# Nicholaswogan/clima

Hardware: AMD Instinct MI355X
Metric: radiate() calls/sec (higher is better)
Workload: dtype f64; 1 GPU; ModernEarth column, one Radtran%radiate call: nz=200, nw=1000 (600 IR + 600 solar bins), 8 g-points, 8 zenith angles, nk=5; config 2 of BASELINE.json; parallelism=1 GPU

## Files before the change

### clima_amd/csrc/radtran_api.hip

```cpp
#include "../../include/clima_radtran_hip.h"
#include "radtran_dev.h"

#include <rccl/rccl.h>
#include <sys/stat.h>
#include <unistd.h>
#include <ctime>

#include <algorithm>
#include <cmath>
#include <cstdio>
#include <cstdlib>
#include <chrono>
#include <cstring>
#include <functional>
#include <set>
#include <string>
#include <utility>
#include <limits>
#include <vector>

using namespace clima;

namespace {

// ... 36 lines not shown
  void alloc(size_t count) {
    release();
    n = count;
    if (count) HIPCHK(hipMalloc((void **)&p, count * sizeof(T)));
  }
  bool reserve(size_t count) {
    const bool grow = n < count;
    if (grow) alloc(count);
    return grow;
  }
  void upload(const std::vector<T> &v) {
    if (!(p && owned && n == v.size())) alloc(v.size());
    if (!v.empty()) HIPCHK(hipMemcpy(p, v.data(), v.size() * sizeof(T), hipMemcpyHostToDevice));
  }
  void zero(hipStream_t s = nullptr) {
    if (n) HIPCHK(hipMemsetAsync(p, 0, n * sizeof(T), s));
  }
  void release() {
    if (p && owned) (void)hipFree(p);
    p = nullptr;
    n = 0;
    owned = true;
  }
  ~DevBuf() { release(); }
};

template <class T>
struct PinnedBuf {
  T *p = nullptr;
  size_t n = 0;
  T *reserve(size_t count, size_t spare = 0) {
    if (n < count) {
      if (p) (void)hipHostFree(p);
      p = nullptr; n = 0;
      HIPCHK(hipHostMalloc((void **)&p, sizeof(T) * (count + spare), hipHostMallocDefault));
      n = count + spare;
    }
    return p;
  }
  ~PinnedBuf() { if (p) (void)hipHostFree(p); }
};

struct KTabHost {
  int sp, ng, nP, nT;
  std::vector<double> weights, log10P, temp, log10k;
  DevBuf<double> d_log10k, d_log10P, d_temp;
// ... 15 lines not shown
  int which = 0;
  int ind_start = 0, ind_end = -1, nw = 0;
  std::vector<double> wavl, freq;
  DevBuf<double> d_freq;
};
struct WrkObj {
  Radtran *parent = nullptr;
  int which = 0;
  DevBuf<double> fup_a, fdn_a, amean, tau_band;
};

struct BatchRun {
  int n = 0, first_call = 0, CH = 0;
  bool one_launch = false, pending = false;
  double *ISR = nullptr, *OLR = nullptr, *fluxes = nullptr;
  double *rows = nullptr;
  const double *bounds = nullptr;
  size_t bounds_count = 0;
  int nsel = 0;
  const int *spec_level = nullptr;
  double *spec[4] = {nullptr, nullptr, nullptr, nullptr};
  double *spec_host = nullptr;
  size_t spec_count = 0;
};

struct Radtran {
  unsigned magic = MAGIC;
  int state = 0;
  int nz = 0, nsp = 0, np = 0, nw = 0, ng = 0;
  std::vector<double> wavl, freq;
  std::vector<KTabHost *> k;
  std::vector<XsHost *> cia, ray, pxs;
  std::vector<PartHost *> part;
  std::vector<int> part_slot;
  bool has_cont = false;
  int LH2O = -1, cont_nT = 0;
  std::vector<double> cont_temp, cont_H2O, cont_foreign;
  DevBuf<double> d_cont_temp, d_cont_H2O, d_cont_foreign;
  std::vector<double> wbin, wbin_e, wxy;
  DevBuf<double> d_wbin, d_wbin_e, d_wbin_e_pad, d_wxy, d_freq, d_rorr_tab;
  ChannelObj ir, sol;
  WrkObj wrk_ir, wrk_sol;
  double diurnal_fac = 0.5;
  std::vector<double> zenith_u, zenith_w, surface_albedo, surface_emissivity, photons_sol;
  bool has_hard_surface = true;
  double ir_tau_min = 1.0e-6;
// ... 70 lines not shown
  DevBuf<double> d_cols_arena, d_flux_arena;
  DevBuf<double> d_prep_arena, d_opr_arena, d_res_arena;
  int batch_cols_in_flight = 64;
  BatchRun dev_batch;
  std::vector<int> spec_level;
  DevBuf<int> d_spec_level;
  DevBuf<double> d_spec_stage;
  PinnedBuf<double> h_spec;
  DevBuf<int> d_batch_nsrc;
  std::vector<int> batch_nsrc;
  hipEvent_t ev_producer = nullptr;
  bool batch_shared = true;
  int rebin_mode = 1;
  bool rebin_stream = false;
  long coop_items = 34816;
  bool fused = true;
  bool ts_block_mode = false;
  DevBuf<int> d_done;
  bool defer_integration = true;
  bool flux_ptr_taken = false;
  bool int_pending = false;
  IntegrateParams pending_ip;
  long merged_integrations = 0, standalone_integrations = 0;
  int profile = 0;
  long timer_calls = 0;
  int profile_stride = 1;
  struct Ev { hipEvent_t a, b; int id; };
  std::vector<Ev> pending;
  std::vector<hipEvent_t> pool;
  double k_ms[7] = {0, 0, 0, 0, 0, 0, 0};
  int k_n[7] = {0, 0, 0, 0, 0, 0, 0};

  ~Radtran() {
    for (auto *x : k) delete x;
    for (auto *x : cia) delete x;
    for (auto *x : ray) delete x;
    for (auto *x : pxs) delete x;
    for (auto *x : part) delete x;
    for (auto &e : pending) { (void)hipEventDestroy(e.a); (void)hipEventDestroy(e.b); }
    for (auto &e : pool) (void)hipEventDestroy(e);
    if (h_col) (void)hipHostFree(h_col);
    for (auto &e : host_registered) (void)hipHostUnregister(e.first);
    for (auto &cs : copy_streams) if (cs) (void)hipStreamDestroy(cs);
    for (auto &e : bout_ev) if (e) (void)hipEventDestroy(e);
    if (h_small) (void)hipHostFree(h_small);
    if (ev_upload) (void)hipEventDestroy(ev_upload);
    if (ev_producer) (void)hipEventDestroy(ev_producer);
    if (comm) (void)ncclCommDestroy(comm);
    if (stream) (void)hipStreamDestroy(stream);
    magic = 0;
  }
};

Radtran *as_rad(void *ptr) {
  Radtran *r = reinterpret_cast<Radtran *>(ptr);
  if (!r || r->magic != MAGIC) return nullptr;
  return r;
}

void gauss_legendre(int n, std::vector<double> &x, std::vector<double> &w) {
  x.assign(n, 0.0);
  w.assign(n, 0.0);
  for (int i = 0; i < n; i++) {
    double z = std::cos(PI * (i + 0.75) / (n + 0.5)), pp = 0.0;
    for (int it = 0; it < 100; it++) {
      double p1 = 1.0, p2 = 0.0;
      for (int j = 0; j < n; j++) {
        double p3 = p2;
        p2 = p1;
        p1 = ((2.0 * j + 1.0) * z * p2 - j * p3) / (j + 1.0);
      }
      pp = n * (z * p1 - p2) / (z * z - 1.0);
      double z1 = z;
      z = z1 - p1 / pp;
      if (std::fabs(z - z1) < 1e-16) break;
    }
    x[n - 1 - i] = z;
    w[n - 1 - i] = 2.0 / ((1.0 - z * z) * pp * pp);
  }
}
// ... 15 lines not shown
  double best1 = INFINITY, best2 = INFINITY;
  for (int i = 0; i < r->nw + 1; i++) {
    double d1 = std::fabs(wavl[0] - r->wavl[i]), d2 = std::fabs(wavl[n - 1] - r->wavl[i]);
    if (d1 < best1) { best1 = d1; ind1 = i; }
    if (d2 < best2) { best2 = d2; ind2 = i; }
  }
  const char *msg = "The wavelength bins are not compatible with the k-distribution wavelength bins.";
  if (n != ind2 - ind1 + 1) { set_err(err, msg); return false; }
  for (int i = 0; i < n; i++)
    if (!is_close(wavl[i], r->wavl[ind1 + i], 1.0e-7)) { set_err(err, msg); return false; }
  c.parent = r;
  c.which = which;
  c.nw = n - 1;
  c.wavl.assign(wavl, wavl + n);
  c.freq.resize(n);
  for (int i = 0; i < n; i++) c.freq[i] = C_LIGHT / (wavl[i] * 1.0e-9);
  c.ind_start = ind1;
  c.ind_end = ind2 - 1;
  return true;
}

void upload_fields(Radtran *r) {
  if (!r->fields_dirty) return;
  if (r->stream) HIPCHK(hipStreamSynchronize(r->stream));
  r->d_zen_u.upload(r->zenith_u);
  r->d_zen_w.upload(r->zenith_w);
  {
    std::vector<double> iu(r->zenith_u.size());
    for (size_t i = 0; i < iu.size(); i++) iu[i] = 1.0 / r->zenith_u[i];
    r->d_zen_iu.upload(iu);
  }
  r->d_albedo.upload(r->surface_albedo);
  r->d_emis.upload(r->surface_emissivity);
  r->d_photons.upload(r->photons_sol);
  r->fields_dirty = false;
}

void weight_edges_and_products(const std::vector<double> &wbin, std::vector<double> &wbin_e, std::vector<double> &wxy) {
  const int ng = (int)wbin.size();
  wbin_e.assign(ng + 1, 0.0);
  for (int i = 1; i < ng + 1; i++) wbin_e[i] = wbin[i - 1] + wbin_e[i - 1];
  wxy.assign((size_t)ng * ng, 0.0);
  for (int i = 0; i < ng; i++)
    for (int j = 0; j < ng; j++) wxy[j + (size_t)i * ng] = wbin[i] * wbin[j];
}

int rebin_mode_for(const std::vector<double> &wbin, const std::vector<double> &wbin_e, const std::vector<double> &wxy, bool stream) {
// ... 372 lines not shown
  if (r->holds.w0_stored) return;
  launch_w0_from_scat(r->d_tau.p, r->d_scat.p, r->d_w0.p, r->nw, r->ng, r->nz, r->stream);
  HIPCHK(hipGetLastError());
  r->holds.w0_formed();
}

bool refuse(const Radtran *r, const char *who, int needs, char *err, bool comm_counts = true) {
  const char *t = refused(r->holds, needs, r->shard_world, comm_counts && r->comm, r->op_lo, r->op_n);
  if (t) set_err(err, t[0] == ' ' ? std::string(who) + t : std::string(t));
  return t != nullptr;
}

bool defer_allowed(bool switch_on, int shard_world, bool has_comm, int profile, bool capturing, bool flux_ptr_taken) {
  return switch_on && shard_world == 1 && !has_comm && profile != 1 && !capturing && !flux_ptr_taken;
}
bool stream_capturing(Radtran *r) {
  hipStreamCaptureStatus st = hipStreamCaptureStatusNone;
  HIPCHK(hipStreamIsCapturing(r->stream, &st));
  return st != hipStreamCaptureStatusNone;
}
bool defer_eligible(Radtran *r) {
  return defer_allowed(r->defer_integration, r->shard_world, r->comm != nullptr, r->profile, false, r->flux_ptr_taken) && !stream_capturing(r);
}
bool resolve_pending_integration(Radtran *r, const PrepParams *prep = nullptr) {
  if (!r->int_pending) return false;
  r->int_pending = false;
  if (prep && r->profile != 1 && prep_integrate_merges(*prep, r->pending_ip) && !stream_capturing(r)) {
    launch_prep_integrate(*prep, r->pending_ip, r->stream);
    HIPCHK(hipGetLastError());
    r->merged_integrations++;
    return true;
  }
  { KernelTimer t(r, 3); launch_integrate(r->pending_ip, r->stream); HIPCHK(hipGetLastError()); t.stop(); }
  r->standalone_integrations++;
  return false;
}

void enqueue_radiate(Radtran *r, const CallBufs &b, bool compute_solar, bool compute_opacity, bool allow_fused = true, bool defer = false) {
  char why[CLIMA_ERR_LEN + 1];
  if (!compute_opacity && refuse(r, "radiate", NEED_OPACITIES, why)) throw HipFail{why};
  r->timer_calls++;
  upload_fields(r);
  const bool resident = b.kind == CALL_RESIDENT, chunk = b.kind == CALL_ARENA_CHUNK;
  const ColumnDev col = column_dev(r, b);
  TwoStreamParams ts = make_twostream_params(r, b, col, compute_solar);
  const LaunchPlan plan = plan_radiate(plan_input(r, b, compute_solar, compute_opacity, allow_fused));
  bool fused_done = false;
  if (compute_opacity) {
    const int call_id = ++r->call_id;
    const PrepParams pp = make_prep_params(r, b, col, call_id, plan.prep_clears ? &ts : nullptr);
    if (!resolve_pending_integration(r, resident && !plan.prep_clears ? &pp : nullptr)) {
      KernelTimer t(r, 0); launch_prep(pp, r->stream); HIPCHK(hipGetLastError()); t.stop();
    }

    OpacityParams op = make_opacity_params(r, b, col, plan.write_w0);
    if (plan.fused.form != TS_NONE) {
      FusedParams fp;
      std::memset(&fp, 0, sizeof(fp));
      fp.ncol = b.ncol; fp.bs = b.bs;
      fp.call_id = call_id; fp.max_spins = r->fused_max_spins;
      fp.done = b.done; fp.timeout_flag = r->d_err.p + 1;
      KernelTimer t(r, 1);
      fused_done = launch_fused(op, ts, fp, plan.fused, r->stream);
      HIPCHK(hipGetLastError());
      t.stop();
      if (!fused_done) op = make_opacity_params(r, b, col, true);
// ... 29 lines not shown
  const IntegrateParams ip = make_integrate_params(r, b, compute_solar, reduce);
  r->holds.rows_enqueued(ip.host_out != nullptr);
  if (defer && resident && !reduce && !ip.host_out && integrate_fits_one_launch(ip.nchunk) && defer_eligible(r)) {
    r->pending_ip = ip;
    r->int_pending = true;
  } else {
    KernelTimer t(r, 3); launch_integrate(ip, r->stream); HIPCHK(hipGetLastError()); t.stop();
  }
  if (reduce) {
    NCCLCHK(ncclAllReduce(r->d_small.p, r->d_small.p, r->rows.reduce_count, ncclDouble, ncclSum, r->comm, r->stream));
    r->comm_reduces++;
  }
}

bool recover_fused_timeout(Radtran *r);
void settle_device_batch(Radtran *r);
void settle_pending_batch(Radtran *r);

void fetch_small(Radtran *r) {
  settle_device_batch(r);
  if (r->holds.rows_on_host) return;
  const LevelRows &l = r->rows;
  for (int pass = 0; pass < 2; pass++) {
    if (!r->holds.rows_in_pinned)
      HIPCHK(hipMemcpyAsync(r->h_small, r->d_small.p, sizeof(double) * l.count, hipMemcpyDeviceToHost, r->stream));
    HIPCHK(hipStreamSynchronize(r->stream));
    resolve_events(r);
    if (r->comm) r->comm_status = r->h_small[l.status];
    if (!r->holds.column || !recover_fused_timeout(r)) break;
  }
  f_total_row(r->h_small, l);
  r->holds.rows_fetched();
}

bool check_dims(Radtran *r, int dim_T, int dim_P, int d1, int d2, int dim_dz, int has_p, int p1, int p2,
                int r1, int r2, const double *pdens, const double *radii, char *err) {
  if (has_p && ((pdens && !radii) || (radii && !pdens))) { set_err(err, "Both pdensities and radii must be arguments."); return false; }
  if (r->np > 0 && (!has_p || !radii)) { set_err(err, "The model contains particles but \"pdensities\" and \"radii\" are not arguments."); return false; }
  if (dim_T != r->nz) { set_err(err, "\"T\" has the wrong input dimension."); return false; }
  if (dim_P != r->nz) { set_err(err, "\"P\" has the wrong input dimension."); return false; }
  if (d1 != r->nz || d2 != r->nsp) { set_err(err, "\"densities\" has the wrong input dimension."); return false; }
  if (dim_dz != r->nz) { set_err(err, "\"dz\" has the wrong input dimension."); return false; }
  if (has_p && radii) {
    if (p1 != r->nz || p2 != r->np) { set_err(err, "\"pdensities\" has the wrong input dimension."); return false; }
    if (r1 != r->nz || r2 != r->np) { set_err(err, "\"radii\" has the wrong input dimension."); return false; }
  }
  return true;
}

void do_upload(Radtran *r, const ColumnArrays &a) {
  const int nz = r->nz;
  double *h = r->h_col;
  settle_pending_batch(r);
  if (r->upload_pending) { HIPCHK(hipEventSynchronize(r->ev_upload)); r->upload_pending = false; }
  r->nsrc = pack_column(r, h, a);
  const int *meta = reinterpret_cast<const int *>(h + r->col_layout.meta);
  bool all = (nz % 2 == 0) && r->nsrc * 2 == nz;
  for (int m = 0; m < r->nsrc && all; m++) all = (meta[1 + m] & SRC_EXACT) != 0;
  r->all_pairs_exact = all;
  if (r->h_col_dev) launch_copy(r->d_col.p, r->h_col_dev, r->col_layout.count, r->stream);
  else HIPCHK(hipMemcpyAsync(r->d_col.p, h, sizeof(double) * r->col_layout.count, hipMemcpyHostToDevice, r->stream));
  HIPCHK(hipEventRecord(r->ev_upload, r->stream));
  r->upload_pending = true;
  r->last_T.assign(a.T, a.T + nz);
  r->last_P.assign(a.P, a.P + nz);
  if (r->np > 0 && a.radii) r->last_radii.assign(a.radii, a.radii + (size_t)nz * r->np); else r->last_radii.clear();
  r->holds.uploaded(a.has_particles());
}

const char *const REPLACED_MSG = "The fused opacity/two-stream hand-off of an earlier opacity pass timed out and the column has "
                                 "been replaced since: repeat the steps from that opacity pass on.";
bool recover_fused_timeout(Radtran *r) {
  if (r->comm) {
    const double st = r->comm_status;
    if (!(st > 0.0)) return false;
    r->comm_status = 0.0;
    r->checked_timeout = r->call_id;
    if (std::fmod(st, 1024.0) > 0.0 && !r->holds.opr_from_resident_column()) throw HipFail{REPLACED_MSG};
    r->fused_fallbacks++;
    enqueue_radiate(r, resident_bufs(r), st >= 1024.0 || r->last_cs, true, false);
    return true;
  }
  const int t = r->h_errflag[1];
  if (t <= r->checked_timeout) return false;
  r->checked_timeout = r->call_id;
  const bool stale_opr = t == r->call_id, stale_sol = t == r->solar_id;
  if (!stale_opr && !stale_sol) return false;
  if (r->shard_world > 1)
    throw HipFail{"The fused opacity/two-stream hand-off timed out on a bin-sharded handle whose all-reduce is the caller's; "
                  "repeat the step (radtran_fused_set(0) selects the separate launches; with radtran_comm_init_rank the "
                  "library repeats it itself)."};
  if (stale_opr && !r->holds.opr_from_resident_column()) throw HipFail{REPLACED_MSG};
  r->fused_fallbacks++;
  enqueue_radiate(r, resident_bufs(r), stale_sol || r->last_cs, true, false);
  return true;
}

constexpr const char *OPACITY_FAILED_MSG = "Opacity computation failed in one or more wavelength bins.";
bool surface_device_error(Radtran *r, char *err) {
  const bool failed = *r->h_errflag > r->checked_id;
  r->checked_id = r->call_id;
  if (failed) set_err(err, OPACITY_FAILED_MSG);
  return failed;
}

void wait_error_words(Radtran *r) {
  HIPCHK(hipMemcpyAsync(r->h_errflag, r->d_err.p, 2 * sizeof(int), hipMemcpyDeviceToHost, r->stream));
  HIPCHK(hipStreamSynchronize(r->stream));
  resolve_events(r);
}

void settle(Radtran *r) {
  settle_device_batch(r);
  for (int pass = 0; pass < 2; pass++) {
    if (r->comm && !r->holds.rows_on_host)
      HIPCHK(hipMemcpyAsync(&r->comm_status, r->d_small.p + r->rows.status, sizeof(double), hipMemcpyDeviceToHost, r->stream));
    wait_error_words(r);
    if (!r->holds.column || !recover_fused_timeout(r)) break;
  }
}

void ready_stored_opacities(Radtran *r) {
  settle(r);
  upload_fields(r);
  ensure_w0(r);
}

void defer_err(Radtran *r, const std::string &msg) {
  if (r && r->deferred_err.empty()) r->deferred_err = msg;
// ... 321 lines not shown
  TRY
  const int nw = r->nw;
  std::vector<double> wv1(nw), row(nwv), tmp(nw);
  for (int i = 0; i < nw; i++) wv1[i] = 0.5 * (r->wavl[i + 1] + r->wavl[i]);
  std::vector<double> tab[3];
  const double *src[3] = {dtau_dz, w0, g0};
  for (auto &t : tab) t.assign((size_t)nw * nP, 0.0);
  for (int i = 0; i < nP; i++) {
    const int j = nP - 1 - i;
    for (int a = 0; a < 3; a++) {
      for (int k = 0; k < nwv; k++) row[k] = src[a][i + (size_t)k * nP];
      if (futils_interp(wv1, nwv, wv, row.data(), tmp.data()) != 0) {
        set_err(err, "Interpolation error in `set_custom_optical_properties`");
        return;
      }
      for (int l = 0; l < nw; l++) tab[a][(size_t)l * nP + j] = tmp[l];
    }
  }
  std::vector<double> lp(nP);
  for (int i = 0; i < nP; i++) lp[nP - 1 - i] = std::log10(P[i]);
  bool ok = nP >= 2;
  for (int i = 1; i < nP && ok; i++) ok = lp[i] > lp[i - 1];
  if (!ok) { set_err(err, "Interpolation initialization error in `set_custom_optical_properties`"); return; }
  HIPCHK(hipStreamSynchronize(r->stream));
  r->cust_axis = lp; r->cust_nP = nP;
  r->d_cust_axis.upload(lp); r->d_cust_dtau.upload(tab[0]); r->d_cust_w0.upload(tab[1]); r->d_cust_g0.upload(tab[2]);
  r->cust_on = true;
  CATCH(err)
}

static std::vector<std::string> split_lines(const char *s) {
  std::vector<std::string> out;
  if (!s) return out;
  std::string cur;
  for (const char *c = s; *c; c++) {
    if (*c == '\n') { out.push_back(cur); cur.clear(); } else cur.push_back(*c);
  }
  if (!cur.empty()) out.push_back(cur);
  return out;
}

void radtran_set_names(void *ptr, const char *species_names, const char *particle_names, char *err) {
  clear_err(err);
  GUARD(r, ptr, err);
  auto sp = split_lines(species_names), pa = split_lines(particle_names);
  if (r->state >= 1 && ((int)sp.size() != r->nsp || (int)pa.size() != r->np)) {
    set_err(err, "radtran_set_names: the number of names does not match the number of species / particles");
// ... 161 lines not shown
      case 8: h.results_dropped(); break;
      default: out[0] = -1; return;
    }
  }
  int k = 0;
  out[k++] = h.column; out[k++] = h.column_particles; out[k++] = (int)h.uploads;
  out[k++] = h.opr; out[k++] = h.w0_stored; out[k++] = (int)h.opr_upload; out[k++] = h.opr_lo; out[k++] = h.opr_n;
  out[k++] = h.rows_on_host; out[k++] = h.rows_in_pinned;
  for (int need : {NEED_COLUMN, NEED_OPACITIES, NEED_SPECTRUM}) out[k++] = refused(h, need, shard_world, has_comm != 0, op_lo, op_n) ? 1 : 0;
  out[k++] = h.opr_from_resident_column();
  static_assert(CLIMA_HOLDS_EVENT_N == 6 && CLIMA_HOLDS_OUT_N == 14, "the orders documented in clima_radtran_hip.h");
}
void clima_test_rebin_mode_for(const int *ng, const double *weights, const int *stream, int *mode) {
  std::vector<double> wbin(weights, weights + std::max(*ng, 0)), wbin_e, wxy;
  if (wbin.empty()) { *mode = -1; return; }
  weight_edges_and_products(wbin, wbin_e, wxy);
  *mode = rebin_mode_for(wbin, wbin_e, wxy, *stream != 0);
}
void radtran_merged_integrations_get(void *ptr, int *merged, int *standalone) {
  Radtran *r = as_rad(ptr);
  *merged = r ? (int)std::min<long>(r->merged_integrations, 2147483647L) : 0;
  *standalone = r ? (int)std::min<long>(r->standalone_integrations, 2147483647L) : 0;
}

void radtran_unset_custom_optical_properties(void *ptr) {
  Radtran *r = as_rad(ptr);
  if (r) r->cust_on = false;
}

void radtran_create_end(void *ptr, const int *num_zenith_angles, const double *surface_albedo, char *err) {
  clear_err(err);
  GUARD(r, ptr, err);
  if (r->state != 1) { set_err(err, "radtran_create_end: create_begin has not been called"); return; }
  if (r->k.empty()) { set_err(err, "There are no k-distributions, yet there must be some to compute total opacity."); return; }
  if (r->ir.nw == 0 || r->sol.nw == 0) { set_err(err, "wavelength channels are not set"); return; }
  if (*num_zenith_angles < 1) { set_err(err, "number of zenith angles must be >= 1"); return; }
  TRY
  const int nz = r->nz, nw = r->nw;
  std::vector<double> x, w;
  gauss_legendre(*num_zenith_angles, x, w);
  r->zenith_u.resize(*num_zenith_angles);
  r->zenith_w.resize(*num_zenith_angles);
  for (int i = 0; i < *num_zenith_angles; i++) {
    double mu = x[i] / 2.0 + 1.0 / 2.0;
    double ang = std::acos(mu) * 180.0 / PI;
    r->zenith_w[i] = w[i] / 2.0;
    r->zenith_u[i] = std::cos(ang * PI / 180.0);
  }
  r->surface_albedo.assign(r->sol.nw, *surface_albedo);
  r->surface_emissivity.assign(r->ir.nw, 1.0);
  if (r->photons_sol.empty()) r->photons_sol.assign(r->sol.nw, 0.0);

  int dev_count = 0;
  HIPCHK(hipGetDeviceCount(&dev_count));
  if (dev_count < 1) throw HipFail{"no HIP device available: the Radtran hot path has no CPU fallback"};
  HIPCHK(hipGetDevice(&r->device));
  HIPCHK(hipStreamCreateWithFlags(&r->stream, hipStreamNonBlocking));
  HIPCHK(hipEventCreateWithFlags(&r->ev_upload, hipEventDisableTiming));

  r->slots.clear();
  auto add_slot = [&](const double *axis_dev, const std::vector<double> &axis, int source, bool flag) {
    SlotDev s;
    s.axis = axis_dev; s.n = (int)axis.size(); s.source = source;
    s.lo = *std::min_element(axis.begin(), axis.end());
    s.hi = *std::max_element(axis.begin(), axis.end());
    s.flag_clamp = flag ? 1 : 0;
    r->slots.push_back(s);
  };
  for (auto *k : r->k) {
    k->d_log10k.upload(k->log10k); k->d_log10P.upload(k->log10P); k->d_temp.upload(k->temp);
    add_slot(k->d_log10P.p, k->log10P, 0, false);
    add_slot(k->d_temp.p, k->temp, 1, false);
  }
  r->abs_entries.clear();
  for (auto *v : {&r->cia, &r->pxs})
    for (auto *xs : *v) {
      xs->d_data.upload(xs->data);
      AbsEntry e;
      e.data = xs->d_data.p; e.nT = xs->dim ? xs->nT : 0; e.slot = 0;
      e.kind = (v == &r->cia) ? ABS_CIA : ABS_COLUMN; e.a = xs->sp1; e.b = xs->sp2 < 0 ? 0 : xs->sp2;
// ... 85 lines not shown
  r->fields_dirty = true;
  compute_shard(r);
  r->holds.rows_fetched();
  r->state = 2;
  CATCH(err)
}

void radtran_upload_column(void *ptr, const double *T_surface, const double *T, const double *P,
                           const double *densities, const double *dz, const double *pdensities,
                           const double *radii, char *err) {
  clear_err(err);
  GUARD_BUILT(r, ptr, err);
  if (r->np > 0 && (!pdensities || !radii)) { set_err(err, "The model contains particles but \"pdensities\" and \"radii\" are not arguments."); return; }
  TRY
  do_upload(r, ColumnArrays{T_surface, T, P, densities, dz, pdensities, radii});
  CATCH(err)
}

void radtran_radiate_resident(void *ptr, const int *compute_solar, const int *compute_opacity, char *err) {
  clear_err(err);
  GUARD_BUILT(r, ptr, err);
  if (refuse(r, "radiate_resident", NEED_COLUMN, err)) return;
  TRY
  enqueue_radiate(r, resident_bufs(r), *compute_solar != 0, *compute_opacity != 0, true, true);
  CATCH(err)
}

static void ir_batch_general(Radtran *r, const double *d_T, const double *d_Ts, int n, double *d_out, size_t out_arr) {
  const int nz = r->nz, nl = nz + 1, nw_ir = r->ir.nw;
  const int CH = std::min(n, 512);
  const int nchunk = integrate_chunks(r->ir_n);
  const size_t spec = (size_t)nw_ir * nl;
  r->d_bup.reserve(spec * CH); r->d_bdn.reserve(spec * CH); r->d_bpartial.reserve((size_t)CH * 2 * nchunk * nl);
  const CallBufs b = resident_bufs(r);
  TwoStreamParams ts = make_twostream_params(r, b, column_dev(r, b), false);
  ts.ir_fup_a = r->d_bup.p; ts.ir_fdn_a = r->d_bdn.p;
  ts.b_T = nz; ts.b_Ts = 1; ts.b_out = spec;
  PlanIn in = plan_input(r, b, false, false, false);
  in.ir_batch = true;
  const LaunchPlan plan = plan_radiate(in);
  for (int c0 = 0; c0 < n; c0 += CH) {
    const int nc = std::min(CH, n - c0);
    TwoStreamParams tb = ts;
    tb.T = d_T + (size_t)c0 * nz; tb.T_surface = d_Ts + c0; tb.b_ncol = nc;
    const bool tiny = nc <= r->batch_shared_min && nz > 256;
    const bool shared_ok = r->batch_shared && !tiny && launch_twostream_ir_batch(tb, nc, r->stream);
    HIPCHK(hipGetLastError());
// ... 1624 lines not shown
  const int zero = 0, one = 1;
  char e[CLIMA_ERR_LEN + 1];
  radtran_set_bin_shard(ptr, &zero, &one, e);
}

void radtran_bin_shard_get(void *ptr, int *op_lo, int *op_n, int *ir_lo, int *ir_n, int *sol_lo, int *sol_n) {
  Radtran *r = as_rad(ptr);
  if (!r) return;
  *op_lo = r->op_lo; *op_n = r->op_n; *ir_lo = r->ir_lo; *ir_n = r->ir_n; *sol_lo = r->sol_lo; *sol_n = r->sol_n;
}

void radtran_finish_reduced(void *ptr, char *err) {
  clear_err(err);
  GUARD_BUILT(r, ptr, err);
  TRY
  settle_device_batch(r);
  CATCH(err)
  r->holds.rows_changed();
}

void radtran_stream_get(void *ptr, void **stream) {
  Radtran *r = as_rad(ptr);
  *stream = r ? (void *)r->stream : nullptr;
}

void radtran_profile_set(void *ptr, const int *enable) {
  Radtran *r = as_rad(ptr);
  if (r) r->profile = (*enable == 2) ? 2 : (*enable != 0 ? 1 : 0);
}
void radtran_profile_stride_set(void *ptr, const int *stride) {
  Radtran *r = as_rad(ptr);
  if (r) r->profile_stride = std::max(1, *stride);
}
void radtran_profile_reset(void *ptr) {
  Radtran *r = as_rad(ptr);
  if (!r) return;
  for (int i = 0; i < 7; i++) { r->k_ms[i] = 0; r->k_n[i] = 0; }
  r->timer_calls = r->profile_stride - 1;
}
void radtran_kernel_time_get(void *ptr, const int *kernel_id, double *ms_total, int *launches, char *err) {
  clear_err(err);
  GUARD(r, ptr, err);
  if (*kernel_id < 0 || *kernel_id > 6) { set_err(err, "kernel id out of range"); return; }
  TRY
  if (!r->pending.empty()) { HIPCHK(hipStreamSynchronize(r->stream)); resolve_events(r); }
  *ms_total = r->k_ms[*kernel_id];
  *launches = r->k_n[*kernel_id];
  CATCH(err)
}

static double distinct_nodes(const std::vector<double> &axis, const std::vector<double> &vals) {
  std::set<int> s;
  const double lo = *std::min_element(axis.begin(), axis.end()), hi = *std::max_element(axis.begin(), axis.end());
  for (double v : vals) { const int i = host_bracket(axis, std::min(std::max(v, lo), hi)); s.insert(i); s.insert(i + 1); }
  return (double)s.size();
}
static double distinct_pt_nodes(const Radtran *r, const KTabHost *k) {
  std::set<std::pair<int, int>> s;
  const double plo = *std::min_element(k->log10P.begin(), k->log10P.end()), phi = *std::max_element(k->log10P.begin(), k->log10P.end());
  const double tlo = *std::min_element(k->temp.begin(), k->temp.end()), thi = *std::max_element(k->temp.begin(), k->temp.end());
  for (int j = 0; j < r->nz; j++) {
    const int iP = host_bracket(k->log10P, std::min(std::max(std::log10(r->last_P[j]), plo), phi));
    const int iT = host_bracket(k->temp, std::min(std::max(r->last_T[j], tlo), thi));
    for (int a = 0; a < 2; a++) for (int b = 0; b < 2; b++) s.insert({iP + a, iT + b});
  }
  return (double)s.size();
}

// ... 582 lines not shown
```

### clima_amd/csrc/radtran_dev.h

```cpp
#pragma once

#include <hip/hip_runtime.h>

#include <cmath>
#include <cstddef>

namespace clima {

constexpr int RB_WIN_LO[8] = {0, 1, 5, 10, 18, 27, 39, 52};
constexpr int RB_WIN_HI[8] = {0, 11, 24, 36, 45, 53, 58, 62};
constexpr int RB_TIGHT_LO[8] = {0, 5, 12, 19, 27, 35, 45, 55};
constexpr int RB_TIGHT_HI[8] = {0, 8, 18, 28, 36, 44, 51, 58};

constexpr int MAX_K = 8;
constexpr int MAX_XS = 16;
constexpr int MAX_PART = 4;
constexpr int MAX_ZEN = 16;
constexpr int MAX_SLOTS = 2 * MAX_K + 2 * MAX_XS + 1 + MAX_PART + 1;

constexpr double PLANK = 6.62607004e-34;
constexpr double C_LIGHT = 299792458.0;
constexpr double K_BOLTZ_SI = 1.380649e-23;
constexpr double PI = 3.14159265358979323846e0;
constexpr double SIGMA_SI = 5.670374419e-8;
// ... 413 lines not shown
  int l0, ir_lo;
  const double *freq, *ir_freq;
  const double *T, *Ts;
  const double *w0, *w1;
  const double *gs0, *gs1;
  const double *gn0, *gn1;
  double *grad_T, *grad_Ts;
};
void launch_ir_rows_vjp(const IrRowsVjpParams &p, hipStream_t s);
int ir_rows_vjp_column_tile(int ncol);
int green_far_resident_waves();
void green_vector_form_set(int vector_form);
int green_far_waves(int ndev, int nl);
int green_far_splits(int n_ir, int waves);

struct Holds {
  bool column = false, column_particles = false;
  long uploads = 0;
  bool opr = false, w0_stored = true;
  long opr_upload = 0;
  int opr_lo = 0, opr_n = 0;
  bool rows_on_host = false, rows_in_pinned = false;
  bool rows = false;

  void uploaded(bool has_particles) { column = true; column_particles = has_particles; uploads++; }
  void opacities_written(bool own_block, bool w0, bool from_resident, int lo, int n) {
    if (!own_block) return;
    opr = true; w0_stored = w0; opr_lo = lo; opr_n = n;
    if (from_resident) opr_upload = uploads;
  }
  void w0_formed() { w0_stored = true; }
  void rows_enqueued(bool in_pinned) { rows = true; rows_on_host = false; rows_in_pinned = in_pinned; }
  void rows_changed() { rows = true; rows_on_host = rows_in_pinned = false; }
  void rows_fetched() { rows_on_host = true; }
  void batch_left(bool one_launch, int np) { column = false; column_particles = np > 0; opr = !one_launch; }
  void batch_repeated() { opr = true; }
  void results_dropped() { rows_changed(); rows = false; opr = false; }
  bool opr_from_resident_column() const { return opr_upload == uploads; }
};
enum { NEED_COLUMN = 1, NEED_OPACITIES = 2, NEED_SPECTRUM = 4 };
inline const char *refused(const Holds &h, int needs, int shard_world, bool has_comm, int op_lo, int op_n) {
  if ((needs & NEED_COLUMN) && !h.column) return "no column has been uploaded";
  if ((needs & NEED_OPACITIES) && !(h.opr && op_lo >= h.opr_lo && op_lo + op_n <= h.opr_lo + h.opr_n))
    return " needs opacities: call radiate with compute_opacity first";
  if ((needs & NEED_SPECTRUM) && shard_world != 1 && !has_comm) return " is not available on a bin-sharded handle";
  return nullptr;
// ... 80 lines not shown
```

### clima_amd/lib.py

```python
import ctypes as C
import os

_HERE = os.path.dirname(os.path.abspath(__file__))
LIB_PATH = os.environ.get("CLIMA_HIP_LIB") or os.path.join(_HERE, "csrc", "libclima_radtran_hip.so")
ERR_LEN = 1024

_dp = C.POINTER(C.c_double)
_ip = C.POINTER(C.c_int)
_bp = C.POINTER(C.c_bool)
_vp = C.c_void_p
_vpp = C.POINTER(C.c_void_p)
_err = C.c_char_p

SIGNATURES = {
    "allocate_radtran": [_vpp],
    "deallocate_radtran": [_vp],
    "radtran_create_begin": [_vp, _ip, _ip, _ip, _ip, _dp, _err],
    "radtran_add_ktable": [_vp, _ip, _ip, _dp, _ip, _dp, _ip, _dp, _dp, _err],
    "radtran_add_xsection": [_vp, _ip, _ip, _ip, _ip, _ip, _dp, _dp, _err],
    "radtran_set_water_continuum": [_vp, _ip, _ip, _dp, _dp, _dp, _err],
    "radtran_add_particle": [_vp, _ip, _ip, _dp, _dp, _dp, _dp, _err],
    "radtran_set_channels": [_vp, _ip, _dp, _ip, _dp, _err],
    "radtran_set_photons_sol": [_vp, _ip, _dp, _err],
    "radtran_create_end": [_vp, _ip, _dp, _err],
    "radtran_radiate_wrapper": [_vp, _dp, _ip, _dp, _ip, _dp, _ip, _ip, _dp, _ip, _dp, _ip, _ip, _ip, _dp, _ip, _ip,
                                _dp, _ip, _ip, _err],
    "radtran_toa_fluxes_wrapper": [_vp, _dp, _ip, _dp, _ip, _dp, _ip, _ip, _dp, _ip, _dp, _ip, _ip, _ip, _dp, _ip, _ip,
                                   _dp, _ip, _ip, _dp, _dp, _err],
    "radtran_apply_radiation_enhancement": [_vp, _dp],
    "radtran_set_custom_optical_properties": [_vp, _ip, _dp, _ip, _dp, _ip, _ip, _dp, _ip, _ip, _dp, _ip, _ip, _dp, _err],
    "radtran_unset_custom_optical_properties": [_vp],
    "radtran_opacities2yaml_wrapper_1": [_vp, _ip, _vpp],
    "radtran_opacities2yaml_wrapper_2": [_vp, _vpp, _ip, _err],
    "radtran_set_names": [_vp, _err, _err, _err],
    "radtran_set_opacity_labels": [_vp, _err, _err, _err, _err],
    "radtran_fused_set": [_vp, _ip],
    "radtran_fused_get": [_vp, _ip],
    "radtran_fused_fallbacks_get": [_vp, _ip],
    "radtran_defer_integration_set": [_vp, _ip],
    "radtran_defer_integration_get": [_vp, _ip],
    "radtran_merged_integrations_get": [_vp, _ip, _ip],
    "clima_test_defer_allowed": [_ip, _ip, _ip, _ip, _ip, _ip, _ip],
    "clima_test_plan_radiate": [_ip, _ip],
    "clima_test_handle_holds": [_ip, _ip, _ip],
    "clima_test_rebin_mode_for": [_ip, _dp, _ip, _ip],
    "radtran_ir_green_set": [_vp, _ip],
    "radtran_ir_green_get": [_vp, _ip, _ip],
    "radtran_coop_items_set": [_vp, _ip],
    "radtran_coop_items_get": [_vp, _ip],
    "radtran_fused_spins_set": [_vp, _ip],
    "radtran_fused_spins_get": [_vp, _ip],
    "radtran_spectra_get_all": [_vp, _bp, _ip, _ip, _ip, _dp, _dp, _dp, _dp, _dp, _dp, _dp, _err],
    "radtran_spectra_release": [_vp],
    "radtran_create_from_files": [_vp, C.c_char_p, C.c_char_p, _ip, _dp, _ip, C.c_char_p, _err],
    "radtran_load_from_files": [_vp, C.c_char_p, C.c_char_p, _ip, C.c_char_p, _err],
    "clima_test_host_tables_digest": [_vp, C.POINTER(C.c_ulonglong)],
    "radtran_dims_get": [_vp, _ip, _ip, _ip, _ip, _ip],
    "radtran_names_get": [_vp, _ip, C.c_char_p, C.c_char_p],
    "radtran_toa_fluxes_batch": [_vp, _ip, _dp, _dp, _dp, _dp, _dp, _ip, _dp, _dp, _dp, _dp, _dp, _err],
    "radtran_toa_fluxes_batch_device": [_vp, _ip, _vp, _vp, _vp, _vp, _vp, _ip, _vp, _vp, _vp, _vp, _vp, _vp, _err],
    "radtran_toa_fluxes_batch_spectra": [_vp, _ip, _dp, _dp, _dp, _dp, _dp, _ip, _dp, _dp, _dp, _dp, _dp, _ip, _ip,
                                         _dp, _dp, _dp, _dp, _err],
    "radtran_toa_fluxes_batch_spectra_device": [_vp, _ip, _vp, _vp, _vp, _vp, _vp, _ip, _vp, _vp, _vp, _vp, _vp, _ip, _ip,
                                                _vp, _vp, _vp, _vp, _vp, _err],
    "radtran_toa_fluxes_batch_bounds": [_vp, _ip, _dp, _dp, _dp, _dp, _dp, _ip, _dp, _dp, _dp, _dp, _dp, _dp, _dp, _dp, _dp, _dp,
# ... 126 lines not shown
```

### clima_amd/radtran.py

```python
import ctypes as C
import os

import numpy as np

from . import lib as _lib

_dp = C.POINTER(C.c_double)


class ClimaException(Exception):
    """clima/cython/_clima.pyx: raised with the Fortran `err` text."""


def _d(a):
    return a.ctypes.data_as(_dp)


def _i(v):
    return C.byref(C.c_int(int(v)))


def _f(v):
    return C.byref(C.c_double(float(v)))

# ... 976 lines not shown
            getattr(self._L, "radtran_%s_set" % name)(self._ptr, C.byref(ctype(to(val))))

        return property(get, set_ if settable else None, doc=doc)

    has_hard_surface = _scalar("has_hard_surface", C.c_bool, bool)
    photon_scale_factor = _scalar("photon_scale_factor", C.c_double, float)
    ir_tau_min = _scalar("ir_tau_min", C.c_double, float)
    diurnal_fac = _scalar("diurnal_fac", C.c_double, float)
    fused = _scalar("fused", C.c_int, bool,
                    "True: opacity + two-stream of a compute_opacity call run as one grid (k_fused).")
    coop_items = _scalar("coop_items", C.c_int, int, "ng = 8: calls with at most this many (bin, source layer) items use "
                         "the group-of-lanes opacity kernel.")
    fused_spins = _scalar("fused_spins", C.c_int, int, "Polls a two-stream block of the fused grid spends waiting for its "
                          "opacity tiles (0: every wait expires and the call is repeated through separate launches).")
    fused_fallbacks = _scalar("fused_fallbacks", C.c_int, int, "Calls re-issued through the separate launches after a fused "
                              "hand-off wait expired.", settable=False)
    ir_green = _scalar("ir_green", C.c_int, int, "radiate_ir_batch's response form: 0 never, 1 (default) when enough columns "
                       "are sparse deviations of one profile, 2 whenever any is.", outs=2)
    ir_green_batches = _scalar("ir_green_batches", C.c_int, int, "Batches that took the response form.", settable=False,
                               getter="ir_green", outs=2, pick=1)
    defer_integration = _scalar("defer_integration", C.c_int, bool, "True (default): a `radiate_resident` call keeps its "
                                "frequency integration back for the next call's prep launch (one grid for both); anything "
                                "that reads results launches it first.  Same results bit for bit.")
    del _scalar

    def _sub(self, name, cls):
        p = C.c_void_p()
        getattr(self._L, "radtran_%s_get" % name)(self._ptr, C.byref(p))
        obj = cls(self._L, p)
        obj._parent = self
        return obj

    ir = property(lambda s: s._sub("ir", RTChannel), doc="RTChannel of the IR bins")
    sol = property(lambda s: s._sub("sol", RTChannel), doc="RTChannel of the solar bins")
    wrk_ir = property(lambda s: s._sub("wrk_ir", ClimaRadtranWrk), doc="IR results")
    wrk_sol = property(lambda s: s._sub("wrk_sol", ClimaRadtranWrk), doc="solar results")
```

### include/clima_radtran_hip.h

```cpp
#ifndef CLIMA_RADTRAN_HIP_H
#define CLIMA_RADTRAN_HIP_H

#ifndef __cplusplus
#include <stdbool.h>
#endif

#ifdef __cplusplus
extern "C" {
#endif

#define CLIMA_ERR_LEN 1024

#define CLIMA_XS_CIA 0
#define CLIMA_XS_RAYLEIGH 1
#define CLIMA_XS_ABSORPTION 2
#define CLIMA_XS_PHOTOLYSIS 3


void allocate_radtran(void **ptr);
void deallocate_radtran(void *ptr);

void radtran_create_begin(void *ptr, const int *nz, const int *nsp, const int *np,
                          const int *nw, const double *wavl, char *err);
void radtran_add_ktable(void *ptr, const int *sp_ind, const int *ngauss,
// ... 161 lines not shown
void radtran_create_from_files(void *ptr, const char *settings_file, const char *star_file, const int *num_zenith_angles,
                               const double *surface_albedo, const int *nz, const char *datadir, char *err);
void radtran_load_from_files(void *ptr, const char *settings_file, const char *star_file, const int *nz, const char *datadir, char *err);
void radtran_dims_get(void *ptr, int *nz, int *nsp, int *np, int *nw, int *ngauss);
void radtran_names_get(void *ptr, const int *cap, char *species_names, char *particle_names);
void radtran_spectra_get_all(void *ptr, const bool *do_solar, const int *nlev, const int *nw_ir, const int *nw_sol,
                             double *ir_fup_a, double *ir_fdn_a, double *ir_tau_band,
                             double *sol_fup_a, double *sol_fdn_a, double *sol_amean, double *sol_tau_band, char *err);
void radtran_spectra_release(void *ptr);
void radtran_batch_pin_results_set(void *ptr, const int *flag);
void radtran_batch_pin_results_get(void *ptr, int *flag);
void radtran_coop_items_set(void *ptr, const int *items);
void radtran_coop_items_get(void *ptr, int *items);
void radtran_fused_spins_set(void *ptr, const int *spins);
void radtran_fused_spins_get(void *ptr, int *spins);
void radtran_ir_green_set(void *ptr, const int *mode);
void radtran_ir_green_get(void *ptr, int *mode, int *batches);
void radtran_fused_fallbacks_get(void *ptr, int *count);
void radtran_defer_integration_set(void *ptr, const int *enable);
void radtran_defer_integration_get(void *ptr, int *enabled);
void radtran_merged_integrations_get(void *ptr, int *merged, int *standalone);
void clima_test_defer_allowed(const int *switch_on, const int *shard_world, const int *has_comm, const int *profile,
                              const int *capturing, const int *flux_ptr_taken, int *allowed);
#define CLIMA_PLAN_IN_N 21
#define CLIMA_PLAN_OUT_N 21
void clima_test_plan_radiate(const int *in, int *out);
#define CLIMA_HOLDS_EVENT_N 6
#define CLIMA_HOLDS_OUT_N 14
void clima_test_handle_holds(const int *n, const int *events, int *out);
void clima_test_rebin_mode_for(const int *ng, const double *weights, const int *stream, int *mode);
void radtran_stream_get(void *ptr, void **stream);
void radtran_profile_set(void *ptr, const int *enable);
void radtran_profile_stride_set(void *ptr, const int *stride);
void radtran_kernel_time_get(void *ptr, const int *kernel_id, double *ms_total, int *launches,
                             char *err);
void radtran_profile_reset(void *ptr);
void radtran_algorithmic_bytes(void *ptr, double *bytes_tables_distinct, double *bytes_in,
                               double *bytes_out, double *bytes_tables_full, char *err);

void radtran_algorithmic_nodes(void *ptr, double *n_pt, double *n_pt_full, double *n_t, double *n_t_full, char *err);

void clima_bench_toa_fluxes(void *ptr, const int *n, const double *T_surface, const int *dim_T, const double *T,
                            const int *dim_P, const double *P, const int *dim1_d, const int *dim2_d,
                            const double *densities, const int *dim_dz, const double *dz, const int *has_particles,
                            const int *dim1_p, const int *dim2_p, const double *pdensities, const int *dim1_r,
                            const int *dim2_r, const double *radii, double *us, double *ISR, double *OLR, char *err);
// ... 83 lines not shown
```

Measured before the change: 11780 calls/s.

## Pipeline consecutive resident radiate calls across two streams and buffer slots

Adds a second set of per-call work buffers and a second stream so that consecutive radiate_resident calls can alternate slots and run concurrently, with events fencing the lanes and the column copy. A heuristic enables this by default when a call's grid exceeds roughly two residency rounds of the device's compute units; a knob forces it on or off. The aim is to hide launch and tail gaps between back-to-back calls, at the cost of doubled buffer memory, extra event and stream synchronisation, and more complex join logic on every result read.

```diff
diff --git a/clima_amd/csrc/radtran_api.hip b/clima_amd/csrc/radtran_api.hip
--- a/clima_amd/csrc/radtran_api.hip
+++ b/clima_amd/csrc/radtran_api.hip
@@ -82,6 +82,7 @@
     n = 0;
     owned = true;
   }
+  void swap(DevBuf &o) { std::swap(p, o.p); std::swap(n, o.n); std::swap(owned, o.owned); }
   ~DevBuf() { release(); }
 };
 
@@ -143,6 +144,15 @@
   double *spec[4] = {nullptr, nullptr, nullptr, nullptr};
   double *spec_host = nullptr;
   size_t spec_count = 0;
+};
+
+struct CallSlot {
+  bool allocated = false;
+  DevBuf<double> d_col, d_prep, d_opr, d_tau, d_w0, d_g, d_tau_band, d_scat;
+  DevBuf<double> spec[8];
+  DevBuf<double> d_small, d_flux_n;
+  DevBuf<int> d_done;
+  long col_upload = 0;
 };
 
 struct Radtran {
@@ -259,6 +269,18 @@
   bool int_pending = false;
   IntegrateParams pending_ip;
   long merged_integrations = 0, standalone_integrations = 0;
+  int calls_in_flight = 0;
+  CallSlot other;
+  long col_upload = 0;
+  hipStream_t lane_stream[2] = {nullptr, nullptr};
+  int lane = 0;
+  bool on_other_lane = false;
+  hipEvent_t ev_lane1 = nullptr;
+  hipEvent_t ev_fence = nullptr;
+  hipEvent_t ev_colcopy = nullptr;
+  bool fence_due = false, colcopy_pending = false;
+  const double *colcopy_src = nullptr;
+  int cus = 0;
   int profile = 0;
   long timer_calls = 0;
   int profile_stride = 1;
@@ -284,6 +306,9 @@
     if (ev_upload) (void)hipEventDestroy(ev_upload);
     if (ev_producer) (void)hipEventDestroy(ev_producer);
     if (comm) (void)ncclCommDestroy(comm);
+    for (hipEvent_t e : {ev_lane1, ev_fence, ev_colcopy}) if (e) (void)hipEventDestroy(e);
+    if (lane_stream[1]) { (void)hipStreamSynchronize(lane_stream[1]); (void)hipStreamDestroy(lane_stream[1]); }
+    if (lane_stream[0]) stream = lane_stream[0];
     if (stream) (void)hipStreamDestroy(stream);
     magic = 0;
   }
@@ -293,6 +318,64 @@
   Radtran *r = reinterpret_cast<Radtran *>(ptr);
   if (!r || r->magic != MAGIC) return nullptr;
   return r;
+}
+
+void join_lanes(Radtran *r) {
+  if (r->on_other_lane) return;
+  if (r->holds.other_in_flight) {
+    HIPCHK(hipEventRecord(r->ev_fence, r->lane_stream[0]));
+    HIPCHK(hipStreamWaitEvent(r->lane_stream[0], r->ev_lane1, 0));
+    r->fence_due = true;
+  }
+  r->holds.joined();
+  r->lane = 0;
+}
+void drain_lanes(Radtran *r) {
+  join_lanes(r);
+  if (r->stream) HIPCHK(hipStreamSynchronize(r->stream));
+}
+struct LaneScope {
+  Radtran *r;
+  int lane;
+  LaneScope(Radtran *r_, int lane_) : r(r_), lane(lane_) {
+    r->on_other_lane = true;
+    r->stream = r->lane_stream[lane];
+    if (lane == 1 && r->fence_due) { r->fence_due = false; HIPCHK(hipStreamWaitEvent(r->stream, r->ev_fence, 0)); }
+  }
+  ~LaneScope() {
+    if (lane == 1) { (void)hipEventRecord(r->ev_lane1, r->lane_stream[1]); r->holds.other_in_flight = true; }
+    r->stream = r->lane_stream[0];
+    r->on_other_lane = false;
+  }
+};
+void ensure_other_slot(Radtran *r) {
+  CallSlot &o = r->other;
+  if (o.allocated) return;
+  if (!r->lane_stream[1]) HIPCHK(hipStreamCreateWithFlags(&r->lane_stream[1], hipStreamNonBlocking));
+  for (hipEvent_t *e : {&r->ev_lane1, &r->ev_fence, &r->ev_colcopy})
+    if (!*e) HIPCHK(hipEventCreateWithFlags(e, hipEventDisableTiming));
+  auto like = [](DevBuf<double> &dst, const DevBuf<double> &src) { dst.alloc(src.n); dst.zero(); };
+  like(o.d_col, r->d_col); like(o.d_prep, r->d_prep); like(o.d_opr, r->d_opr);
+  auto view = [&](DevBuf<double> &dst, const DevBuf<double> &src) { dst.view(o.d_opr.p + (src.p - r->d_opr.p), src.n); };
+  view(o.d_tau, r->d_tau); view(o.d_w0, r->d_w0); view(o.d_g, r->d_g); view(o.d_tau_band, r->d_tau_band); view(o.d_scat, r->d_scat);
+  const DevBuf<double> *spec[8] = {&r->wrk_ir.fup_a, &r->wrk_ir.fdn_a, &r->wrk_ir.amean, &r->wrk_ir.tau_band,
+                                   &r->wrk_sol.fup_a, &r->wrk_sol.fdn_a, &r->wrk_sol.amean, &r->wrk_sol.tau_band};
+  for (int k = 0; k < 8; k++) like(o.spec[k], *spec[k]);
+  o.d_small.alloc(r->rows.count); o.d_small.zero();
+  o.d_flux_n.view(o.d_small.p, r->rows.flux_count);
+  o.d_done.alloc(r->d_done.n); o.d_done.zero();
+  HIPCHK(hipStreamSynchronize(nullptr));
+  o.allocated = true;
+}
+void swap_slot(Radtran *r) {
+  CallSlot &o = r->other;
+  r->d_col.swap(o.d_col); r->d_prep.swap(o.d_prep); r->d_opr.swap(o.d_opr);
+  r->d_tau.swap(o.d_tau); r->d_w0.swap(o.d_w0); r->d_g.swap(o.d_g); r->d_tau_band.swap(o.d_tau_band); r->d_scat.swap(o.d_scat);
+  DevBuf<double> *spec[8] = {&r->wrk_ir.fup_a, &r->wrk_ir.fdn_a, &r->wrk_ir.amean, &r->wrk_ir.tau_band,
+                             &r->wrk_sol.fup_a, &r->wrk_sol.fdn_a, &r->wrk_sol.amean, &r->wrk_sol.tau_band};
+  for (int k = 0; k < 8; k++) spec[k]->swap(o.spec[k]);
+  r->d_small.swap(o.d_small); r->d_flux_n.swap(o.d_flux_n); r->d_done.swap(o.d_done);
+  std::swap(r->col_upload, o.col_upload);
 }
 
 void gauss_legendre(int n, std::vector<double> &x, std::vector<double> &w) {
@@ -354,7 +437,7 @@
 
 void upload_fields(Radtran *r) {
   if (!r->fields_dirty) return;
-  if (r->stream) HIPCHK(hipStreamSynchronize(r->stream));
+  drain_lanes(r);
   r->d_zen_u.upload(r->zenith_u);
   r->d_zen_w.upload(r->zenith_w);
   {
@@ -773,7 +856,43 @@
 bool defer_eligible(Radtran *r) {
   return defer_allowed(r->defer_integration, r->shard_world, r->comm != nullptr, r->profile, false, r->flux_ptr_taken) && !stream_capturing(r);
 }
+long radiate_grid_waves(const PlanIn &in, const LaunchPlan &pl) {
+  const long items = (long)in.op_n * in.nsrc, tiles = (items + 255) / 256;
+  if (pl.fused.form != TS_NONE) return 4 * (tiles + (long)(in.n_sol + in.n_ir) * pl.fused.groups);
+  if (pl.opacity == OP_COOP) return 4 * ((items * pl.coop_ng + 255) / 256);
+  return 4 * tiles;
+}
+struct TwoInFlight {
+  int mode;
+  bool defer_ok, prev_unjoined, sampled, fields_dirty, int_pending, integrates_in_one_launch;
+  long grid_waves;
+  int cus;
+};
+bool two_in_flight_allowed(const TwoInFlight &q) {
+  if (q.mode == 1 || !q.defer_ok || !q.prev_unjoined || q.sampled || q.fields_dirty || q.int_pending || !q.integrates_in_one_launch) return false;
+  return q.mode == 2 || q.grid_waves > 2L * 4 * q.cus;
+}
+bool call_is_sampled(const Radtran *r) {
+  return r->profile == 2 && (r->profile_stride <= 1 || (r->timer_calls + 1) % r->profile_stride == 0);
+}
+bool two_in_flight(Radtran *r, bool prev_unjoined, bool int_pending) {
+  TwoInFlight q{};
+  q.mode = r->calls_in_flight; q.prev_unjoined = prev_unjoined; q.int_pending = int_pending;
+  q.sampled = call_is_sampled(r); q.fields_dirty = r->fields_dirty; q.cus = r->cus;
+  q.defer_ok = defer_allowed(r->defer_integration, r->shard_world, r->comm != nullptr, r->profile, false, r->flux_ptr_taken);
+  q.integrates_in_one_launch = integrate_fits_one_launch(integrate_chunks(std::max(r->ir_n, r->sol_n)));
+  if (q.mode == 0 && q.defer_ok && prev_unjoined) {
+    const PlanIn in = plan_input(r, resident_bufs(r, false), true, true, true);
+    q.grid_waves = radiate_grid_waves(in, plan_radiate(in));
+  }
+  if (!two_in_flight_allowed(q)) return false;
+  q.defer_ok = !stream_capturing(r);
+  return two_in_flight_allowed(q);
+}
+bool pipelining_two(Radtran *r) { return two_in_flight(r, true, false); }
+
 bool resolve_pending_integration(Radtran *r, const PrepParams *prep = nullptr) {
+  join_lanes(r);
   if (!r->int_pending) return false;
   r->int_pending = false;
   if (prep && r->profile != 1 && prep_integrate_merges(*prep, r->pending_ip) && !stream_capturing(r)) {
@@ -787,12 +906,31 @@
   return false;
 }
 
+void wait_for_column_copy(Radtran *r, const double *block_to_write) {
+  if (!r->colcopy_pending || r->colcopy_src != block_to_write) return;
+  HIPCHK(hipStreamWaitEvent(r->stream, r->ev_colcopy, 0));
+  r->colcopy_pending = false;
+}
+void ensure_column(Radtran *r) {
+  if (r->col_upload == r->holds.uploads || !r->other.allocated || r->other.col_upload != r->holds.uploads) return;
+  if (r->upload_pending) HIPCHK(hipStreamWaitEvent(r->stream, r->ev_upload, 0));
+  wait_for_column_copy(r, r->d_col.p);
+  if (r->colcopy_pending) HIPCHK(hipStreamWaitEvent(r->stream, r->ev_colcopy, 0));
+  launch_copy(r->d_col.p, r->other.d_col.p, r->col_layout.count, r->stream);
+  HIPCHK(hipGetLastError());
+  HIPCHK(hipEventRecord(r->ev_colcopy, r->stream));
+  r->colcopy_pending = true;
+  r->colcopy_src = r->other.d_col.p;
+  r->col_upload = r->holds.uploads;
+}
+
 void enqueue_radiate(Radtran *r, const CallBufs &b, bool compute_solar, bool compute_opacity, bool allow_fused = true, bool defer = false) {
   char why[CLIMA_ERR_LEN + 1];
   if (!compute_opacity && refuse(r, "radiate", NEED_OPACITIES, why)) throw HipFail{why};
   r->timer_calls++;
   upload_fields(r);
   const bool resident = b.kind == CALL_RESIDENT, chunk = b.kind == CALL_ARENA_CHUNK;
+  if (resident) { join_lanes(r); ensure_column(r); }
   const ColumnDev col = column_dev(r, b);
   TwoStreamParams ts = make_twostream_params(r, b, col, compute_solar);
   const LaunchPlan plan = plan_radiate(plan_input(r, b, compute_solar, compute_opacity, allow_fused));
@@ -868,8 +1006,11 @@
   if (r->holds.rows_on_host) return;
   const LevelRows &l = r->rows;
   for (int pass = 0; pass < 2; pass++) {
-    if (!r->holds.rows_in_pinned)
-      HIPCHK(hipMemcpyAsync(r->h_small, r->d_small.p, sizeof(double) * l.count, hipMemcpyDeviceToHost, r->stream));
+    if (!r->holds.rows_in_pinned) {
+      const bool own = reinterpret_cast<int *>(r->d_small.p + l.err_words) == r->d_err.p;
+      HIPCHK(hipMemcpyAsync(r->h_small, r->d_small.p, sizeof(double) * (own ? l.count : l.err_words), hipMemcpyDeviceToHost, r->stream));
+      if (!own) HIPCHK(hipMemcpyAsync(r->h_errflag, r->d_err.p, 2 * sizeof(int), hipMemcpyDeviceToHost, r->stream));
+    }
     HIPCHK(hipStreamSynchronize(r->stream));
     resolve_events(r);
     if (r->comm) r->comm_status = r->h_small[l.status];
@@ -904,9 +1045,17 @@
   bool all = (nz % 2 == 0) && r->nsrc * 2 == nz;
   for (int m = 0; m < r->nsrc && all; m++) all = (meta[1 + m] & SRC_EXACT) != 0;
   r->all_pairs_exact = all;
-  if (r->h_col_dev) launch_copy(r->d_col.p, r->h_col_dev, r->col_layout.count, r->stream);
-  else HIPCHK(hipMemcpyAsync(r->d_col.p, h, sizeof(double) * r->col_layout.count, hipMemcpyHostToDevice, r->stream));
-  HIPCHK(hipEventRecord(r->ev_upload, r->stream));
+  const bool to_other = r->holds.unjoined && pipelining_two(r);
+  if (to_other) ensure_other_slot(r); else join_lanes(r);
+  {
+    LaneScope lane(r, to_other ? r->lane ^ 1 : 0);
+    double *d_col = to_other ? r->other.d_col.p : r->d_col.p;
+    wait_for_column_copy(r, d_col);
+    if (r->h_col_dev) launch_copy(d_col, r->h_col_dev, r->col_layout.count, r->stream);
+    else HIPCHK(hipMemcpyAsync(d_col, h, sizeof(double) * r->col_layout.count, hipMemcpyHostToDevice, r->stream));
+    HIPCHK(hipEventRecord(r->ev_upload, r->stream));
+    (to_other ? r->other.col_upload : r->col_upload) = r->holds.uploads + 1;
+  }
   r->upload_pending = true;
   r->last_T.assign(a.T, a.T + nz);
   r->last_P.assign(a.P, a.P + nz);
@@ -951,6 +1100,7 @@
 }
 
 void wait_error_words(Radtran *r) {
+  join_lanes(r);
   HIPCHK(hipMemcpyAsync(r->h_errflag, r->d_err.p, 2 * sizeof(int), hipMemcpyDeviceToHost, r->stream));
   HIPCHK(hipStreamSynchronize(r->stream));
   resolve_events(r);
@@ -1318,7 +1468,7 @@
   bool ok = nP >= 2;
   for (int i = 1; i < nP && ok; i++) ok = lp[i] > lp[i - 1];
   if (!ok) { set_err(err, "Interpolation initialization error in `set_custom_optical_properties`"); return; }
-  HIPCHK(hipStreamSynchronize(r->stream));
+  drain_lanes(r);
   r->cust_axis = lp; r->cust_nP = nP;
   r->d_cust_axis.upload(lp); r->d_cust_dtau.upload(tab[0]); r->d_cust_w0.upload(tab[1]); r->d_cust_g0.upload(tab[2]);
   r->cust_on = true;
@@ -1526,6 +1676,35 @@
   *merged = r ? (int)std::min<long>(r->merged_integrations, 2147483647L) : 0;
   *standalone = r ? (int)std::min<long>(r->standalone_integrations, 2147483647L) : 0;
 }
+void radtran_calls_in_flight_set(void *ptr, const int *mode) {
+  Radtran *r = as_rad(ptr);
+  if (r) r->calls_in_flight = std::max(0, std::min(2, *mode));
+}
+void radtran_calls_in_flight_get(void *ptr, int *mode) {
+  Radtran *r = as_rad(ptr);
+  *mode = r ? r->calls_in_flight : 0;
+}
+void radtran_overlapped_calls_get(void *ptr, int *count) {
+  Radtran *r = as_rad(ptr);
+  *count = r ? (int)std::min<long>(r->holds.overlapped, 2147483647L) : 0;
+}
+void clima_test_two_in_flight(const int *rule, const int *in, int *out) {
+  PlanIn p{};
+  p.nz = in[0]; p.ng = in[1]; p.nzen = in[2]; p.n_ir = in[3]; p.n_sol = in[4]; p.op_n = in[5]; p.nsrc = in[6]; p.ncol = in[7];
+  p.batch = in[8] != 0; p.ir_batch = in[9] != 0; p.rebin_mode = in[10]; p.cust_on = in[11] != 0;
+  p.compute_opacity = in[12] != 0; p.all_pairs = in[13] != 0; p.fused = in[14] != 0; p.allow_fused = in[15] != 0;
+  p.ts_block_mode = in[16] != 0; p.no_half = in[17] != 0; p.coop_items = in[18]; p.force_slots = in[19];
+  const long waves = radiate_grid_waves(p, plan_radiate(p));
+  TwoInFlight q{};
+  q.mode = rule[0];
+  q.defer_ok = defer_allowed(rule[1] != 0, rule[2], rule[3] != 0, rule[4], rule[5] != 0, rule[6] != 0);
+  q.prev_unjoined = rule[7] != 0; q.sampled = rule[8] != 0; q.cus = rule[9];
+  q.fields_dirty = rule[10] != 0; q.int_pending = rule[11] != 0; q.integrates_in_one_launch = integrate_fits_one_launch(integrate_chunks(in[20]));
+  q.grid_waves = waves;
+  out[0] = two_in_flight_allowed(q) ? 1 : 0;
+  out[1] = (int)std::min<long>(waves, 2147483647L);
+  static_assert(CLIMA_TWO_IN_FLIGHT_RULE_N == 12, "the order documented in clima_radtran_hip.h");
+}
 
 void radtran_unset_custom_optical_properties(void *ptr) {
   Radtran *r = as_rad(ptr);
@@ -1560,6 +1739,8 @@
   if (dev_count < 1) throw HipFail{"no HIP device available: the Radtran hot path has no CPU fallback"};
   HIPCHK(hipGetDevice(&r->device));
   HIPCHK(hipStreamCreateWithFlags(&r->stream, hipStreamNonBlocking));
+  r->lane_stream[0] = r->stream;
+  HIPCHK(hipDeviceGetAttribute(&r->cus, hipDeviceAttributeMultiprocessorCount, r->device));
   HIPCHK(hipEventCreateWithFlags(&r->ev_upload, hipEventDisableTiming));
 
   r->slots.clear();
@@ -1691,7 +1872,28 @@
   GUARD_BUILT(r, ptr, err);
   if (refuse(r, "radiate_resident", NEED_COLUMN, err)) return;
   TRY
-  enqueue_radiate(r, resident_bufs(r), *compute_solar != 0, *compute_opacity != 0, true, true);
+  const bool cs = *compute_solar != 0, co = *compute_opacity != 0;
+  upload_fields(r);
+  const bool beside = cs && co && two_in_flight(r, r->holds.unjoined, r->int_pending);
+  const bool two = beside || (cs && co && pipelining_two(r));
+  if (beside) {
+    ensure_other_slot(r);
+    swap_slot(r);
+    r->lane ^= 1;
+    try {
+      LaneScope lane(r, r->lane);
+      enqueue_radiate(r, resident_bufs(r), cs, co, true, false);
+    } catch (...) {
+      swap_slot(r);
+      r->lane ^= 1;
+      r->holds.other_in_flight = true;
+      throw;
+    }
+    r->holds.call_pipelined(true);
+  } else {
+    enqueue_radiate(r, resident_bufs(r), cs, co, true, !two);
+    if (two) r->holds.call_pipelined(false);
+  }
   CATCH(err)
 }
 
@@ -3362,6 +3564,8 @@
 void radtran_stream_get(void *ptr, void **stream) {
   Radtran *r = as_rad(ptr);
   *stream = r ? (void *)r->stream : nullptr;
+  if (!r || r->state != 2) return;
+  try { join_lanes(r); } catch (const HipFail &f) { defer_err(r, f.msg); }
 }
 
 void radtran_profile_set(void *ptr, const int *enable) {
@@ -3383,7 +3587,7 @@
   GUARD(r, ptr, err);
   if (*kernel_id < 0 || *kernel_id > 6) { set_err(err, "kernel id out of range"); return; }
   TRY
-  if (!r->pending.empty()) { HIPCHK(hipStreamSynchronize(r->stream)); resolve_events(r); }
+  if (!r->pending.empty()) { drain_lanes(r); resolve_events(r); }
   *ms_total = r->k_ms[*kernel_id];
   *launches = r->k_n[*kernel_id];
   CATCH(err)
diff --git a/clima_amd/csrc/radtran_dev.h b/clima_amd/csrc/radtran_dev.h
--- a/clima_amd/csrc/radtran_dev.h
+++ b/clima_amd/csrc/radtran_dev.h
@@ -459,6 +459,14 @@
   int opr_lo = 0, opr_n = 0;
   bool rows_on_host = false, rows_in_pinned = false;
   bool rows = false;
+  bool other_in_flight = false, unjoined = false;
+  long overlapped = 0;
+
+  void call_pipelined(bool took_other) {
+    if (took_other) { other_in_flight = true; overlapped++; }
+    unjoined = true;
+  }
+  void joined() { other_in_flight = false; unjoined = false; }
 
   void uploaded(bool has_particles) { column = true; column_particles = has_particles; uploads++; }
   void opacities_written(bool own_block, bool w0, bool from_resident, int lo, int n) {
diff --git a/clima_amd/lib.py b/clima_amd/lib.py
--- a/clima_amd/lib.py
+++ b/clima_amd/lib.py
@@ -41,6 +41,10 @@
     "radtran_defer_integration_get": [_vp, _ip],
     "radtran_merged_integrations_get": [_vp, _ip, _ip],
     "clima_test_defer_allowed": [_ip, _ip, _ip, _ip, _ip, _ip, _ip],
+    "radtran_calls_in_flight_set": [_vp, _ip],
+    "radtran_calls_in_flight_get": [_vp, _ip],
+    "radtran_overlapped_calls_get": [_vp, _ip],
+    "clima_test_two_in_flight": [_ip, _ip, _ip],
     "clima_test_plan_radiate": [_ip, _ip],
     "clima_test_handle_holds": [_ip, _ip, _ip],
     "clima_test_rebin_mode_for": [_ip, _dp, _ip, _ip],
diff --git a/clima_amd/radtran.py b/clima_amd/radtran.py
--- a/clima_amd/radtran.py
+++ b/clima_amd/radtran.py
@@ -1022,6 +1022,12 @@
     defer_integration = _scalar("defer_integration", C.c_int, bool, "True (default): a `radiate_resident` call keeps its "
                                 "frequency integration back for the next call's prep launch (one grid for both); anything "
                                 "that reads results launches it first.  Same results bit for bit.")
+    calls_in_flight = _scalar("calls_in_flight", C.c_int, int, "Pipelined `radiate_resident` calls in flight: 0 (default) two "
+                              "where a call's grid does not fit the device in one residency round, 1 one at a time, 2 two "
+                              "whenever eligible.  Consecutive calls alternate between two sets of work buffers and two "
+                              "streams; everything else joins first.  Same results bit for bit.")
+    overlapped_calls = _scalar("overlapped_calls", C.c_int, int, "Calls enqueued on one call slot while the other slot's "
+                               "call had not been joined.", settable=False)
     del _scalar
 
     def _sub(self, name, cls):
diff --git a/include/clima_radtran_hip.h b/include/clima_radtran_hip.h
--- a/include/clima_radtran_hip.h
+++ b/include/clima_radtran_hip.h
@@ -207,6 +207,11 @@
 void radtran_merged_integrations_get(void *ptr, int *merged, int *standalone);
 void clima_test_defer_allowed(const int *switch_on, const int *shard_world, const int *has_comm, const int *profile,
                               const int *capturing, const int *flux_ptr_taken, int *allowed);
+void radtran_calls_in_flight_set(void *ptr, const int *mode);
+void radtran_calls_in_flight_get(void *ptr, int *mode);
+void radtran_overlapped_calls_get(void *ptr, int *count);
+#define CLIMA_TWO_IN_FLIGHT_RULE_N 12
+void clima_test_two_in_flight(const int *rule, const int *in, int *out);
 #define CLIMA_PLAN_IN_N 21
 #define CLIMA_PLAN_OUT_N 21
 void clima_test_plan_radiate(const int *in, int *out);
```

Measured after the change: 13270 calls/s (median of 6 runs). 1.13x the previous value.
